# tudoroancea/ihm2

Hardware: AMD Instinct MI355X
Metric: NMPC RTI solves/s (batch), N=40, nx=8 (6-DOF bicycle), fkin6 (higher is better)
Workload: dtype f64

## Files before the change

### ihm2_amd/csrc/kernels_qp.hip

```cpp
#include <cstring>

#include "ihm2mpc_internal.h"
#include "device_steps.hpp"
#include "sqp_body.hpp"
#include "irk_body.hpp"
#include "riccati_mfma.hpp"
#include "sens_body.hpp"
#include "qp_lds.hpp"
#include "qp_mrows.hpp"
#include "qp_reduce.hpp"
#include "qp_catalogue.hpp"
#include "wave_sync.hpp"

using namespace ihm2;

namespace {

#define INF_BOUND 1e20
#ifndef RIC_RING
#define RIC_RING 4
#endif
#ifndef SWEEP_RING
#define SWEEP_RING 4
#endif
#define SWEEP_DL ((SWEEP_RING >= 8) ? 4 : 2)

__device__ __forceinline__ bool fin(double v) { return fabs(v) < INF_BOUND; }
__device__ __forceinline__ int here(int v) { asm volatile("" : "+v"(v)); return v; }

template <typename OP>
__device__ __forceinline__ double wave_reduce(double v, OP op)
{
    v = op(v, dpp_mov<0xB1>(v));
    v = op(v, dpp_mov<0x4E>(v));
    v = op(v, dpp_mov<0x141>(v));
    v = op(v, dpp_mov<0x128>(v));
    int lo = __double2loint(v), hi = __double2hiint(v);
    auto a16 = __builtin_amdgcn_permlane16_swap(lo, lo, false, false);
    auto b16 = __builtin_amdgcn_permlane16_swap(hi, hi, false, false);
    v = op(__hiloint2double(b16[0], a16[0]), __hiloint2double(b16[1], a16[1]));
    lo = __double2loint(v); hi = __double2hiint(v);
    auto a32 = __builtin_amdgcn_permlane32_swap(lo, lo, false, false);
    auto b32 = __builtin_amdgcn_permlane32_swap(hi, hi, false, false);
    return op(__hiloint2double(b32[0], a32[0]), __hiloint2double(b32[1], a32[1]));
}
__device__ __forceinline__ double nanmax(double a, double b) { return (a != a || b != b) ? NAN : fmax(a, b); }
__device__ __forceinline__ double wave_max(double v) { return wave_reduce(v, [](double a, double b) { return fmax(a, b); }); }
__device__ __forceinline__ double wave_min(double v) { return wave_reduce(v, [](double a, double b) { return fmin(a, b); }); }
__device__ __forceinline__ double wave_sum(double v) { return wave_reduce(v, [](double a, double b) { return a + b; }); }
__device__ __forceinline__ double wave_nanmax(double v) { return wave_reduce(v, [](double a, double b) { return nanmax(a, b); }); }
__device__ __forceinline__ void norm_max(double &res, bool &bad, double v) { bad |= v != v; res = fmax(res, v); }

__device__ __forceinline__ double sum8(double v)
{
    v += dpp_mov<0xB1>(v);
    v += dpp_mov<0x4E>(v);
    v += dpp_mov<0x141>(v);
    return v;
}

__device__ __forceinline__ double sum_stride8(double v)
{
    v += dpp_mov<0x128>(v);
// ... 48 lines not shown
                    }
                }
            }
        }
        return;
    }
    double r[2][D], x0[DL], x1[DL];
    const __amdgpu_buffer_rsrc_t rsrc = __builtin_amdgcn_make_buffer_rsrc(const_cast<double *>(rows) - (size_t)QM_PAD * 64, 0, (N + 2 * QM_PAD) * 512, 0x00020000);
    const unsigned ve = (unsigned)e_even * 8u, vo = (unsigned)e_odd * 8u;
    typedef unsigned int u2_t __attribute__((ext_vector_type(2)));
    const double *p_even = rows + (size_t)((DIR < 0) ? N - 1 : 0) * 64 + e_even, *p_odd = rows + (size_t)((DIR < 0) ? N - 1 : 0) * 64 + e_odd;
    auto load_row = [&](const int step, const bool odd) -> double {
        if constexpr (BUF) {
            const int row = (DIR < 0) ? N - 1 - step : step;
            const u2_t v = __builtin_amdgcn_raw_buffer_load_b64(rsrc, odd ? vo : ve, (QM_PAD + row) * 512, 0);
            return __hiloint2double((int)v.y, (int)v.x);
        } else
            return (odd ? p_odd : p_even)[(ptrdiff_t)DIR * step * 64];
    };
#pragma unroll
    for (int d = 0; d < D; d++) {
        r[0][d] = load_row(d, (d & 1) != 0);
        __builtin_amdgcn_sched_barrier(0);
        if (d < DL) pre((DIR < 0) ? N - 1 - d : d, (d & 1) != 0, x0[d], x1[d]);
    }
    for (int s0 = 0; s0 < N; s0 += 2 * D) {
#pragma unroll
        for (int h = 0; h < 2; h++) {
#pragma unroll
            for (int d = 0; d < D; d++) {
                const int s = s0 + h * D + d;
                const int k = (DIR < 0) ? N - 1 - s : s;
                const double v = r[h][d], y0 = x0[d % DL], y1 = x1[d % DL];
                r[h ^ 1][d] = load_row(s + D, (d & 1) != 0);
                pre((DIR < 0) ? k - DL : k + DL, (d & 1) != 0, x0[d % DL], x1[d % DL]);
                if (s < N) body(k, v, (d & 1) != 0, y0, y1);
            }
        }
    }
}
template <int DIR, int D, int DL, typename P, typename F>
__device__ __forceinline__ void stream_rows_v1(const double *rows, int N, int e_even, int e_odd, P &&pre, F &&body)
{
    stream_rows<DIR, D, DL, false>(rows, N, e_even, e_odd, pre, body);
}

template <int NSLOT, int NSOFT, int PATH, int UNI, int NW = 1, int LEAN = 1, int NF = 0, int FULL = 0>
__device__ __forceinline__ void qp_wave_body(const QpArgs &a, const int b, double *sm, const bool want_res = true)
{
    static_assert(NF == 0 || NW == 1, "the straight-line factor sweep parks its idle lanes' stores in the tile the block reductions use");
    static_assert(FULL == 0 || (NSOFT == 0 && PATH == 0 && UNI != 0 && NW == 1 && LEAN != 0 && NF > 0 && NSLOT <= 8),
                  "the full slot form is written for the all-hard table of the batch-shared rows, one wave, the lean phases and the compiled-in horizon");
    constexpr int NT = 64 * NW;
    constexpr bool PAIRM = NF > 0;
    static_assert(!PAIRM || (NF % 4 == 0 && LEAN != 0 && NW == 1 && qm_pair_inside(NF > 0 ? NF : 2, SWEEP_RING, QM_PAD)),
                  "the paired rows: an even horizon in whole factor passes, the lean sweeps, and their unclamped prefetch inside q_M's padding");
    const int tid = threadIdx.x, lane = tid & 63, wv = tid >> 6;
#define BSYNC() do { if (NW == 1) WSYNC(); else __syncthreads(); } while (0)
    const int N = (NF > 0) ? NF : a.N, NS = N + 1;
    constexpr QpLdsClass CLS = qp_lds_class(PATH, UNI != 0);
    constexpr int NCK = CLS.nck;
    const double *Hs0 = a.Hs + (size_t)b * a.hs_bs, *HsT = Hs0 + a.hs_te;
    const double *Gy0 = a.Gy + (size_t)b * a.gy_bs, *GyT = Gy0 + a.gy_te;
    const double *slot_lbb = a.slot_lb + (size_t)b * a.sl_bs, *slot_ubb = a.slot_ub + (size_t)b * a.sl_bs;
    constexpr bool ALAT = PATH == 2;
    constexpr bool HL = CLS.hl, CL = CLS.cl;
    static_assert(qp_factor_inside(qp_lds(40, CLS), 40, NCK) && qp_factor_inside(qp_lds(2, CLS), 2, NCK), "factor stage / block reductions leave their LDS");
    static_assert(qp_sweeps_inside(qp_lds(40, CLS), 40, LEAN != 0, SWEEP_RING, SWEEP_DL) && (LEAN == 0 || qp_sweeps_inside(qp_lds(2, CLS), 2, true, SWEEP_RING, SWEEP_DL)),
                  "the sweeps' unclamped LDS prefetch leaves the block (the earlier form does below N = 4: api.hip refuses those launches)");
    static_assert(NW <= 4, "qp_factor_inside checks the block reductions for four waves");
    static_assert(FULL == 0 || qp_full_zeroes_kept(qp_lds(NF > 0 ? NF : 2, CLS), NF > 0 ? NF : 2), "a store of the factor sweep reaches gam or cf: the full slot form zeroes them once per solve");
#define LEN(id) qp_lds_len(id, N, NS, CLS)
    double *z = sm, *gt = z + LEN(QP_Z), *pi = gt + LEN(QP_GT), *pv = pi + LEN(QP_PI), *rb = pv + LEN(QP_PV), *gam = rb + LEN(QP_RB), *cf = gam + LEN(QP_GAM), *dz = cf + LEN(QP_CF);
    double *kff = dz + LEN(QP_DZ), *Kl = kff + LEN(QP_KFF), *Ginv = Kl + LEN(QP_KL), *Prb = Ginv + LEN(QP_GINV), *tile = Prb + LEN(QP_PRB), *hc = tile + LEN(QP_TILE), *ha = hc + LEN(QP_HC);
    double *Hl = ha + LEN(QP_HA), *CDl = Hl + LEN(QP_HL), *spv = CDl + LEN(QP_CDL);
    int *spc = reinterpret_cast<int *>(spv + 60);
#undef LEN
#define HS(k, i, l) (HL ? Hl[(((k) == N) ? 100 : 0) + (i) * 10 + (l)] : ((k) == N ? HsT : Hs0 + (UNI ? 0 : (k)) * 100)[(i) * 10 + (l)])
#define CDV(k, r, j) (CL ? CDl[(r) * 10 + (j)] : a.CD[((k) * 2 + (r)) * 10 + (j)])

    auto blk_reduce = [&](double v, auto op) -> double {
        v = wave_reduce(v, op);
        if (NW > 1) {
            __syncthreads();
            if (lane == 0) tile[wv] = v;
            __syncthreads();
            v = tile[0];
#pragma unroll
            for (int w = 1; w < NW; w++) v = op(v, tile[w]);
        }
        return v;
    };
    auto blk_max = [&](double v) { return blk_reduce(v, [](double x, double y) { return fmax(x, y); }); };
    auto blk_min = [&](double v) { return blk_reduce(v, [](double x, double y) { return fmin(x, y); }); };
    auto blk_sum = [&](double v) { return blk_reduce(v, [](double x, double y) { return x + y; }); };
    auto blk_nanmax = [&](double v) { return blk_reduce(v, [](double x, double y) { return nanmax(x, y); }); };

    const double *xb = a.x + (size_t)b * NS * 8;
    const double *ub = a.u + (size_t)b * N * 2;
    const double *linb = a.lin + (size_t)b * N * LIN_REC;
    double *gb = a.g + (size_t)b * NS * 10;
    double *rgb = a.rg + (size_t)b * NS * 10;
    double *Pg = a.P + (size_t)b * NS * 64;
    double *Mg = a.M + (size_t)b * N * 64;
    double *pib = a.pi + (size_t)b * NS * 8;
    double *lamb = a.lam + (size_t)b * NS * 28;
// ... 71 lines not shown
            st = fma(-CDV(k, 0, j), lamb[k * 28 + 10] - lamb[k * 28 + 24], st);
            st = fma(-CDV(k, 1, j), lamb[k * 28 + 11] - lamb[k * 28 + 25], st);
        }
        if (PATH && (j == 1 || j == 2)) {
            const double l12 = lamb[k * 28 + 12] - lamb[k * 28 + 26], l13 = lamb[k * 28 + 13] - lamb[k * 28 + 27];
            st -= (j == 1) ? l12 - l13 : hc[k * 2] * l12 + hc[k * 2 + 1] * l13;
        }
        if (ALAT && alat_slot(j) >= 0) st -= ha[k * 4 + alat_slot(j)] * (lamab[k * 2] - lamab[k * 2 + 1]);
        if (counted) r_stat = fmax(r_stat, fabs(st));
    }
    for (int e = tid; e < N * 8; e += NT) {
        const double bl = linb[(size_t)(e / 8) * LIN_REC + 80 + (e % 8)];
        sb = fmax(sb, fabs(bl));
        r_eq = fmax(r_eq, fabs(bl));
    }
    if (tid < 8) {
        const double d = a.x0[(size_t)b * 8 + tid] - xb[tid];
        sb = fmax(sb, fabs(d));
        r_eq = fmax(r_eq, fabs(d));
    }
    if constexpr (FULL != 0) { double sg2 = sg, sb2 = sb; wave_max4(lane, sg, sb, sg2, sb2); }
    else { sg = blk_max(sg); sb = blk_max(sb); }

    int s_kc[NSLOT];
    double s_dl[NSLOT], s_du[NSLOT];
    double lam_l[NSLOT], lam_u[NSLOT], t_l[NSLOT], t_u[NSLOT];
    constexpr int NSO = (NSOFT > 0) ? NSOFT : 1;
    double so_zw[NSO], so_Zw[NSO], so_s[NSO], so_ls[NSO], so_rs[NSO], so_ds[NSO], so_dls[NSO], so_pa[NSO];
#pragma unroll
    for (int r = 0; r < NSO; r++) { so_zw[r] = 0.0; so_Zw[r] = -1.0; so_s[r] = 1.0; so_ls[r] = 0.0; so_rs[r] = 0.0; so_ds[r] = so_dls[r] = so_pa[r] = 0.0; }
#define IS_SOFT(r) ((r) < NSOFT && so_Zw[(r) < NSOFT ? (r) : 0] >= 0.0)
#define ONE_SIDED(r) (NSOFT > 0 && PATH != 2 && (r) < NSOFT)
#define HAS_L(r) (FULL ? true : ONE_SIDED(r) ? true : fin(s_dl[r]))
#define HAS_U(r) (FULL ? true : ONE_SIDED(r) ? false : fin(s_du[r]))
#define ROW_DOT(r, v) (FULL ? row_dot_full((r), (v)) : ONE_SIDED(r) ? s_sg[(r) < NSOFT ? (r) : 0] * row_dot(s_kc[r], (v)) : row_dot(s_kc[r], (v)))
#define NO_SLOT(r) (!FULL && s_kc[r] < 0)
#define SLOT_W(r) (FULL ? (s_kc[r] & 0xffff) >> 3 : s_kc[r])
#define SLOT_AT(arr, r) (*(FULL ? reinterpret_cast<double *>(reinterpret_cast<char *>(arr) + (here(s_kc[r]) & 0xffff)) : &(arr)[s_kc[r]]))
#define ROW_SIGN(r, c) (ONE_SIDED(r) ? s_sg[(r) < NSOFT ? (r) : 0] * (c) : (c))
    double s_sg[NSO];
#pragma unroll
    for (int r = 0; r < NSO; r++) s_sg[r] = 1.0;
#define SLOT_ACC(dst, v) do { if (NSOFT > 0) (dst) += (v); else (dst) = (v); } while (0)
    double r_ineq = 0.0, r_comp = 0.0;
#pragma unroll
    for (int r = 0; r < NSLOT; r++) {
        const int s = tid + NT * r;
        s_kc[r] = FULL ? 0 : -1; s_dl[r] = -INFINITY; s_du[r] = INFINITY;
        lam_l[r] = lam_u[r] = 0.0; t_l[r] = t_u[r] = 1.0;
        const int kc = (s < a.nslots) ? a.slot_kc[s] : -1;
        if (kc >= 0) {
            const int k = kc >> 4, c = kc & 15;
            s_kc[r] = k * NCK + c;
            if (FULL) s_kc[r] = ((k * NCK + c) * 8) | ((k * 10 + ((c < 10) ? c : 0)) << 19) | ((c >= 10) ? (int)(0x80000000u | ((unsigned)(c - 10) << 30)) : 0);
            double cz;
            if (c < 8) cz = xb[k * 8 + c];
            else if (c < 10) cz = ub[k * 2 + c - 8];
            else if (ALAT && c == 14) {
                double g4[4];
                cz = alat_eval(xb[k * 8 + 3], xb[k * 8 + 4], xb[k * 8 + 6], xb[k * 8 + 7], g4);
            } else if (c >= 12) {
                const double n = xb[k * 8 + 1], psi = xb[k * 8 + 2];
                const double foot = -0.5 * a.car_L * sin(fabs(psi)), lat = 0.5 * a.car_W * cos(psi);
                cz = (c == 12) ? n + foot + lat - w_R : -n - foot + lat - w_L;
            } else {
                cz = 0.0;
#pragma unroll
                for (int j = 0; j < 8; j++) cz = fma(CDV(k, c - 10, j), xb[k * 8 + j], cz);
                cz = fma(CDV(k, c - 10, 8), ub[k * 2 + 0], cz);
                cz = fma(CDV(k, c - 10, 9), ub[k * 2 + 1], cz);
            }
            const double lb = slot_lbb[s], ubd = slot_ubb[s];
            bool soft = false;
            if (r < NSOFT) { so_zw[r < NSOFT ? r : 0] = a.slot_zw[s]; so_Zw[r < NSOFT ? r : 0] = a.slot_Zw[s]; soft = a.slot_Zw[s] >= 0.0; }
#define LAM_IN(up) ((ALAT && c == 14) ? lamab[k * 2 + (up)] : lamb[k * 28 + 14 * (up) + c])
            if (fin(lb)) { s_dl[r] = lb - cz; if (want_res && !soft) { r_ineq = fmax(r_ineq, s_dl[r]); r_comp = fmax(r_comp, fabs(LAM_IN(0) * s_dl[r])); } }
            if (fin(ubd)) { s_du[r] = ubd - cz; if (want_res && !soft) { r_ineq = fmax(r_ineq, -s_du[r]); r_comp = fmax(r_comp, fabs(LAM_IN(1) * s_du[r])); } }
#undef LAM_IN
            if (ONE_SIDED(r) && fin(ubd)) { s_sg[r < NSOFT ? r : 0] = -1.0; s_dl[r] = -s_du[r]; }
        }
    }
    if (want_res) {
        if constexpr (FULL != 0) wave_max4(lane, r_stat, r_eq, r_ineq, r_comp);
        else { r_stat = blk_max(r_stat); r_eq = blk_max(r_eq); r_ineq = blk_max(r_ineq); r_comp = blk_max(r_comp); }
    }
    if (want_res && tid == 0) {
        double *rs = a.res + (size_t)b * 4;
        rs[0] = r_stat; rs[1] = r_eq; rs[2] = r_ineq; rs[3] = r_comp;
    }

    const double tol_g = a.tol * sg, tol_b = a.tol * sb, tol_d = a.tol * sb, tol_m = a.tol * sg;
    const double mu_floor = 0.1 * tol_m;
    const double mu0 = a.mu0 * sg;
    const double inv_m = (a.m_act > 0) ? 1.0 / a.m_act : 0.0;

    auto row_dot = [&](int kc, const double *v) -> double {
        const int k = kc / NCK, c = kc % NCK;
        if (c < 10) return v[k * 10 + c];
        if (ALAT && c == 14) return ha[k * 4] * v[k * 10 + 3] + ha[k * 4 + 1] * v[k * 10 + 4] + ha[k * 4 + 2] * v[k * 10 + 6] + ha[k * 4 + 3] * v[k * 10 + 7];
        if (PATH && c >= 12) return (c == 12) ? v[k * 10 + 1] + hc[k * 2] * v[k * 10 + 2] : -v[k * 10 + 1] + hc[k * 2 + 1] * v[k * 10 + 2];
        double acc = 0.0;
#pragma unroll
        for (int j = 0; j < 10; j++) acc = fma(CDV(k, c - 10, j), v[k * 10 + j], acc);
        return acc;
    };
    auto row_dot_full = [&](int r, const double *v) -> double {
        const int pk = here(s_kc[r]);
        const double *vk = reinterpret_cast<const double *>(reinterpret_cast<const char *>(v) + ((pk >> 16) & 0x3fff));
        if (pk >= 0) return vk[0];
        const double *cd = CDl + (((unsigned)pk >> 30) & 1) * 10;
        double acc = 0.0;
#pragma unroll
        for (int j = 0; j < 10; j++) acc = fma(cd[j], vk[j], acc);
        return acc;
    };

    for (int e = tid; e < NS * 10; e += NT) z[e] = (e < 8) ? a.x0[(size_t)b * 8 + e] - xb[e] : 0.0;
    for (int e = tid; e < NS * 8; e += NT) pi[e] = 0.0;
    if (FULL) for (int e = tid; e < NS * NCK; e += NT) { cf[e] = 0.0; gam[e] = 0.0; }
    BSYNC();
#pragma unroll
    for (int r = 0; r < NSLOT; r++) {
        if (NO_SLOT(r)) continue;
        const double rz = ROW_DOT(r, z);
        const bool al = HAS_L(r), au = HAS_U(r);
        double tau_c = a.tau0;
        if (al && au) tau_c = fmin(a.tau0, 0.25 * (s_du[r] - s_dl[r]));
        if (IS_SOFT(r)) {
            const double slack = al ? rz - s_dl[r] : s_du[r] - rz;
            const double s0 = fmax(a.tau0, a.tau0 - slack);
            so_s[r < NSOFT ? r : 0] = s0;
            so_ls[r < NSOFT ? r : 0] = mu0 / s0;
            if (al) { t_l[r] = slack + s0; lam_l[r] = mu0 / t_l[r]; } else { t_u[r] = slack + s0; lam_u[r] = mu0 / t_u[r]; }
            continue;
        }
        if (al) { t_l[r] = fmax(rz - s_dl[r], tau_c); lam_l[r] = mu0 / t_l[r]; }
        if (au) { t_u[r] = fmax(s_du[r] - rz, tau_c); lam_u[r] = mu0 / t_u[r]; }
    }

    int qstatus = 1, it = 0;
    bool exact_mode = false;
    double res_g = 0, res_b = 0, res_d = 0, res_m = 0, mu = 0;
    double fol_g = 0.0, fol_b = 0.0;
    double rd_l[NSLOT], rd_u[NSLOT], dlam_l[NSLOT], dlam_u[NSLOT], dt_l[NSLOT], dt_u[NSLOT];
    double pa_l[NSLOT], pa_u[NSLOT];
    for (it = 0;; it++) {
        bool exact = (it == 0) || exact_mode, finished = false;
        auto multipliers_to_cf = [&]() {
            if (!FULL) {
                for (int e = tid; e < NS * NCK; e += NT) cf[e] = 0.0;
                BSYNC();
            }
#pragma unroll
            for (int r = 0; r < NSLOT; r++) {
                if (NO_SLOT(r)) continue;
                const bool al = HAS_L(r), au = HAS_U(r);
                SLOT_ACC(SLOT_AT(cf, r), ROW_SIGN(r, (al ? lam_l[r] : 0.0) - (au ? lam_u[r] : 0.0)));
            }
            BSYNC();
        };
        if (LEAN != 0) { if (exact) multipliers_to_cf(); }
        else {
            for (int e = tid; e < NS * NCK; e += NT) cf[e] = 0.0;
            BSYNC();
        }
        double mu_acc = 0.0, res_gs = 0.0;
        res_d = 0.0; res_m = 0.0;
        double lane_d = 0.0, lane_m = 0.0;
        bool bad_d = false, bad_m = false, bad_gs = false;
#pragma unroll
        for (int r = 0; r < NSLOT; r++) {
            rd_l[r] = rd_u[r] = 0.0;
            if (NO_SLOT(r)) continue;
            const double rz = ROW_DOT(r, z);
            const bool al = HAS_L(r), au = HAS_U(r);
            const double sv = IS_SOFT(r) ? so_s[r < NSOFT ? r : 0] : 0.0;
            double pl = 0.0, pu = 0.0;
            if constexpr (FULL != 0) {
                rd_l[r] = rz - t_l[r] - s_dl[r] + sv; pl = __dmul_rn(lam_l[r], t_l[r]); norm_max(lane_m, bad_m, fabs(pl));
                rd_u[r] = s_du[r] - rz - t_u[r] + sv; pu = __dmul_rn(lam_u[r], t_u[r]); norm_max(lane_m, bad_m, fabs(pu));
            } else {
            if (al) { rd_l[r] = rz - t_l[r] - s_dl[r] + sv; pl = __dmul_rn(lam_l[r], t_l[r]); res_m = nanmax(res_m, fabs(pl)); }
            if (au) { rd_u[r] = s_du[r] - rz - t_u[r] + sv; pu = __dmul_rn(lam_u[r], t_u[r]); res_m = nanmax(res_m, fabs(pu)); }
            }
            mu_acc = __dadd_rn(mu_acc, __dadd_rn(pl, pu));
            if constexpr (FULL != 0) { bad_d |= __builtin_isunordered(rd_l[r], rd_u[r]); lane_d = fmax(lane_d, fmax(fabs(rd_l[r]), fabs(rd_u[r]))); }
            else
            res_d = nanmax(res_d, nanmax(fabs(rd_l[r]), fabs(rd_u[r])));
            if (IS_SOFT(r)) {
                const int q = r < NSOFT ? r : 0;
                so_rs[q] = so_Zw[q] * so_s[q] + so_zw[q] - (al ? lam_l[r] : lam_u[r]) - so_ls[q];
                if constexpr (FULL != 0) {
                    norm_max(res_gs, bad_gs, fabs(so_rs[q]));
                    mu_acc += so_ls[q] * so_s[q]; norm_max(lane_m, bad_m, fabs(so_ls[q] * so_s[q]));
                } else {
                res_gs = nanmax(res_gs, fabs(so_rs[q]));
                mu_acc += so_ls[q] * so_s[q]; res_m = nanmax(res_m, fabs(so_ls[q] * so_s[q]));
                }
            }
            if (LEAN == 0) SLOT_ACC(SLOT_AT(cf, r), ROW_SIGN(r, (al ? lam_l[r] : 0.0) - (au ? lam_u[r] : 0.0)));
        }
        if constexpr (NW > 1) {
#pragma unroll
            for (int r = 0; r < NSLOT; r++) {
                const int sidx = tid + NT * r;
                if (sidx >= a.nslots_can) continue;
                const bool on = s_kc[r] >= 0;
                gam[sidx] = __dadd_rn((on && fin(s_dl[r])) ? __dmul_rn(lam_l[r], t_l[r]) : 0.0, (on && fin(s_du[r])) ? __dmul_rn(lam_u[r], t_u[r]) : 0.0);
            }
            __syncthreads();
            mu_acc = 0.0;
            for (int sidx = lane; sidx < a.nslots_can; sidx += 64) mu_acc = __dadd_rn(mu_acc, gam[sidx]);
            __syncthreads();
        }
        if (LEAN == 0) BSYNC();
        for (int rpass = 0; rpass < 2; rpass++) {
            if (exact) {
                for (int e = tid; e < NS * 10; e += NT) {
                    const int k = e / 10, j = e % 10;
                    double acc = gb[e];
                    if (HL && h_sparse) {
                        const int row = ((k == N) ? 10 : 0) + j;
// ... 13 lines not shown
                        const double l12 = cf[k * NCK + 12], l13 = cf[k * NCK + 13];
                        acc -= (j == 1) ? l12 - l13 : hc[k * 2] * l12 + hc[k * 2 + 1] * l13;
                    }
                    if (ALAT && alat_slot(j) >= 0) acc -= ha[k * 4 + alat_slot(j)] * cf[k * NCK + 14];
                    gt[e] = acc;
                }
                BSYNC();
                dyn_residual<4, NT>(N, tid, const_cast<double *>(linb), z, pi, gt, rb, LIN_REC);
                BSYNC();
            }
            res_g = 0.0; res_b = 0.0;
            if (exact || LEAN == 0) {
                for (int e = tid; e < NS * 10; e += NT) {
                    const int k = e / 10, j = e % 10;
                    double v = gt[e];
                    if ((k == 0 && j < 8) || (k == N && j >= 8)) { v = 0.0; gt[e] = 0.0; }
                    if (exact) rgb[e] = v;
                    res_g = nanmax(res_g, fabs(v));
                }
                for (int e = tid; e < N * 8; e += NT) res_b = nanmax(res_b, fabs(rb[e]));
            } else { res_g = fol_g; res_b = fol_b; }
            if constexpr (FULL != 0) {
                const bool nan_g = wave_any(res_g != res_g || bad_gs), nan_b = wave_any(res_b != res_b), nan_d = wave_any(bad_d), nan_m = wave_any(bad_m);
                res_g = fmax(res_g, res_gs);
                res_d = lane_d; res_m = lane_m;
                wave_max4(lane, res_g, res_b, res_d, res_m);
                mu = wave_sum(mu_acc) * inv_m;
                res_g = nan_g ? NAN : res_g; res_b = nan_b ? NAN : res_b; res_d = nan_d ? NAN : res_d; res_m = nan_m ? NAN : res_m;
            } else {
            res_g = nanmax(res_g, res_gs);
            res_g = blk_nanmax(res_g); res_b = blk_nanmax(res_b);
            if (rpass == 0) { res_d = blk_nanmax(res_d); res_m = blk_nanmax(res_m); mu = ((NW == 1) ? blk_sum(mu_acc) : wave_sum(mu_acc)) * inv_m; }
            }
            if (!(res_g == res_g) || !(res_b == res_b) || !(res_d == res_d) || !(res_m == res_m)) { qstatus = (it == 0) ? 3 : 4; finished = true; break; }
            const bool conv = res_g <= tol_g && res_b <= tol_b && res_d <= tol_d && res_m <= tol_m;
            if (conv && exact) { qstatus = 0; finished = true; break; }
            if ((conv || it >= a.iter_max) && !exact) {
                exact = true; exact_mode = true;
                if (LEAN != 0) multipliers_to_cf();
                continue;
            }
            break;
        }
        if (finished) break;
        if (it >= a.iter_max) { qstatus = 1; break; }
        BSYNC();
        double alpha = 1.0, alpha_d = 1.0, sigma = 0.0;
        auto slot_coeffs = [&](int pass) {
            if (!FULL) {
                for (int e = tid; e < NS * NCK; e += NT) { cf[e] = 0.0; if (pass == 0) gam[e] = 0.0; }
                BSYNC();
            }
            const double mu_t = fmax(sigma * mu, mu_floor);
#pragma unroll
            for (int r = 0; r < NSLOT; r++) {
                if (NO_SLOT(r)) continue;
                const bool al = HAS_L(r), au = HAS_U(r);
                double c = 0.0;
                if (IS_SOFT(r)) {
                    const int q = r < NSOFT ? r : 0;
                    const double lm = al ? lam_l[r] : lam_u[r], tt = al ? t_l[r] : t_u[r], rdv = al ? rd_l[r] : rd_u[r];
                    const double gm = lm / tt, gs = so_ls[q] / so_s[q], D = so_Zw[q] + gm + gs;
                    double c1, c2, rsv;
                    if (pass == 0) { c1 = (lm * tt + lm * rdv) / tt; c2 = so_ls[q]; rsv = so_rs[q]; SLOT_AT(gam, r) += gm * (so_Zw[q] + gs) / D; }
                    else { c1 = ((al ? pa_l[r] : pa_u[r]) - mu_t) / tt; c2 = (so_pa[q] - mu_t) / so_s[q]; rsv = 0.0; }
                    c = c1 - gm * (rsv + c1 + c2) / D;
                    SLOT_AT(cf, r) += ONE_SIDED(r) ? ROW_SIGN(r, c) : (al ? c : -c);
                    continue;
                }
                if (pass == 0) {
                    const double gl = al ? lam_l[r] / t_l[r] : 0.0, gu = au ? lam_u[r] / t_u[r] : 0.0;
                    if (al) c += fma(gl, rd_l[r], lam_l[r]);
                    if (au) c -= fma(gu, rd_u[r], lam_u[r]);
                    SLOT_ACC(SLOT_AT(gam, r), gl + gu);
                } else {
                    if (al) c += (pa_l[r] - mu_t) / t_l[r];
                    if (au) c -= (pa_u[r] - mu_t) / t_u[r];
                }
                SLOT_ACC(SLOT_AT(cf, r), ROW_SIGN(r, c));
            }
            BSYNC();
        };
        auto add_coeffs = [&]() {
            for (int e = tid; e < NS * 10; e += NT) {
                const int k = e / 10, j = e % 10;
                double acc = gt[e] + cf[k * NCK + j];
                if (k < N) {
                    acc = fma(CDV(k, 0, j), cf[k * NCK + 10], acc);
                    acc = fma(CDV(k, 1, j), cf[k * NCK + 11], acc);
                }
                if (PATH && (j == 1 || j == 2)) {
                    const double c12 = cf[k * NCK + 12], c13 = cf[k * NCK + 13];
                    acc += (j == 1) ? c12 - c13 : hc[k * 2] * c12 + hc[k * 2 + 1] * c13;
                }
                if (ALAT && alat_slot(j) >= 0) acc += ha[k * 4 + alat_slot(j)] * cf[k * NCK + 14];
                gt[e] = acc;
            }
            BSYNC();

        };
        slot_coeffs(0);
        add_coeffs();
        __builtin_amdgcn_s_waitcnt(0x0F70);
        if (wv == 0) {
            RicLds L;
            const QpRic o = qp_lds_ric(N, NS, NCK);
            L.gt = o.gt; L.pv = o.pv; L.gam = o.gam; L.dz = o.dz; L.kff = o.kff; L.Kl = o.Kl;
            L.Ginv = o.Ginv; L.hv = o.Prb; L.tile = o.tile; L.hc = o.hc; L.ha = o.ha;
            if constexpr (NF != 0)
                riccati_sweep_mfma<NCK, PATH != 0, UNI != 0, RIC_RING, ALAT, true, (NF > 0) ? NF : 0>(N, lane, linb, Hs0, HsT, a.CD, L, Pg, Mg, LIN_REC, false, false);
            else
            riccati_sweep_mfma<NCK, PATH != 0, UNI != 0, RIC_RING, ALAT>(N, lane, linb, Hs0, HsT, a.CD, L, Pg, Mg, LIN_REC, a.m_act == 0, a.symmetrize != 0);
            if (lane < 8) dz[lane] = 0.0;
        }
        BSYNC();
        for (int pass = 0; pass < 2; pass++) {
            const double mu_t = fmax(sigma * mu, mu_floor);
            if (pass == 1) slot_coeffs(1);
            if (pass == 1) {
            add_coeffs();
            for (int e = tid; e < NS * 8; e += NT) {
                const int k = e >> 3, j = e & 7;
                double v = gt[k * 10 + j];
                if (k < N) v -= Kl[k * 16 + j] * gt[k * 10 + 8] + Kl[k * 16 + 8 + j] * gt[k * 10 + 9];
                pv[e] = v;
            }
            BSYNC();
            if constexpr (LEAN != 0) {
            if (wv == 0) {
                const int g = lane >> 3, w = lane & 7;
                double pw = pv[N * 8 + w], pg = 0.0;
                const int se2 = (w == 0) ? 16 : 0, so2 = (g == 0) ? 16 : 0;
                const double *be = (w == 0) ? pv + (N - 1) * 8 + g : dz, *bo = (g == 0) ? pv + (N - 2) * 8 + w : dz;
                const double *qe = Prb + (N - 1) * 8 + w, *qo = Prb + (N - 2) * 8 + g;
                double *oe = pv + (N - 1) * 8 + g, *oo = pv + (N - 2) * 8 + w;
                stream_rows<-1, SWEEP_RING, SWEEP_DL, true, PAIRM>(Mg, N, RIC_IDX(w, g), RIC_IDX(g, w),
                    [&](int k, bool odd, double &prb, double &base) {
                        if (odd) { prb = *qo; qo -= 16; base = *bo; bo -= so2; } else { prb = *qe; qe -= 16; base = *be; be -= se2; }
                    },
                    [&](int k, double m, bool odd, double prb, double base) {
                        if (!odd) {
                            pg = sum8(fma(m, pw, fma(m, prb, base)));
                            *oe = pg; oe -= 16;
                        } else {
                            pw = sum_stride8(fma(m, pg, fma(m, prb, base)));
                            *oo = pw; oo -= 16;
                        }
                    });
            }
            } else {
            if (wv == 0) {
                const int g = lane >> 3, w = lane & 7;
                double pw = pv[N * 8 + w], pg = 0.0;
                stream_rows_v1<-1, QP_V1_RING, QP_V1_DL>(Mg, N, RIC_IDX(w, g), RIC_IDX(g, w),
                    [&](int k, bool odd, double &prb, double &base) { prb = Prb[k * 8 + (odd ? g : w)]; base = pv[k * 8 + (odd ? w : g)]; },
                    [&](int k, double m, bool odd, double prb, double base) {
                        if (!odd) {
                            const double off = fma(m, prb, (w == 0) ? base : 0.0);
                            pg = sum8(fma(m, pw, off));
                            if (w == 0) pv[k * 8 + g] = pg;
                        } else {
                            const double off = fma(m, prb, (g == 0) ? base : 0.0);
                            pw = sum_stride8(fma(m, pg, off));
                            if (g == 0) pv[k * 8 + w] = pw;
                        }
                    });
            }
            }
// ... 44 lines not shown
            }
            } else {
            if (wv == 0) {
                const int g = lane >> 3, w = lane & 7;
                double dxw = dz[w], dxg = 0.0;
                stream_rows_v1<+1, QP_V1_RING, QP_V1_DL>(Mg, N, RIC_IDX(g, w), RIC_IDX(w, g),
                    [&](int k, bool odd, double &c, double &unused) { c = dz[(k + 1) * 10 + (odd ? w : g)]; unused = 0.0; },
                    [&](int k, double m, bool odd, double c, double) {
                        if (!odd) {
                            dxg = sum8(fma(m, dxw, (w == 0) ? c : 0.0));
                            if (w == 0) dz[(k + 1) * 10 + g] = dxg;
                        } else {
                            dxw = sum_stride8(fma(m, dxg, (g == 0) ? c : 0.0));
                            if (g == 0) dz[(k + 1) * 10 + w] = dxw;
                        }
                    });
            }
            }
            BSYNC();
            const bool want_dpi = (pass == 1) || (a.m_act == 0);
            for (int e = tid; e < NS * 2; e += NT) {
                const int k = e >> 1, aa = e & 1;
                double acc = 0.0;
                if (k < N) {
                    acc = -kff[k * 4 + aa];
#pragma unroll
                    for (int l = 0; l < 8; l++) acc = fma(-Kl[k * 16 + aa * 8 + l], dz[k * 10 + l], acc);
                }
                dz[k * 10 + 8 + aa] = acc;
            }
            if (want_dpi) {
                const int n = NS * 8;
                for (int base = 0; base < n; base += 3 * NT) {
                    double2 pr[3][4];
#pragma unroll
                    for (int q = 0; q < 3; q++) {
                        const int e = min(base + NT * q + tid, n - 1), k = e >> 3, i = e & 7;
#pragma unroll
                        for (int l = 0; l < 4; l++) pr[q][l] = *reinterpret_cast<const double2 *>(Pg + (size_t)k * 64 + RIC_IDX(l, i));
                    }
#pragma unroll
                    for (int q = 0; q < 3; q++) {
                        const int e = base + NT * q + tid, ec = min(e, n - 1), k = ec >> 3;
                        double acc = pv[ec];
#pragma unroll
                        for (int l = 0; l < 4; l++) { acc = fma(pr[q][l].x, dz[k * 10 + l], acc); acc = fma(pr[q][l].y, dz[k * 10 + l + 4], acc); }
                        if (e < n) pv[e] = acc;
                    }
                }
            }
            BSYNC();

            double amax = 1.0, amax_d = 1.0, mu_aff = 0.0, rmax = 1.0, rmax_d = 1.0;
#pragma unroll
            for (int r = 0; r < NSLOT; r++) {
                dlam_l[r] = dlam_u[r] = dt_l[r] = dt_u[r] = 0.0;
                if (NO_SLOT(r)) continue;
                const double drz = ROW_DOT(r, dz);
                if (IS_SOFT(r)) {
                    const int q = r < NSOFT ? r : 0;
                    const bool al = HAS_L(r);
                    const double lm = al ? lam_l[r] : lam_u[r], tt = al ? t_l[r] : t_u[r], rdv = al ? rd_l[r] : rd_u[r];
                    const double y = al ? drz : -drz;
                    const double gm = lm / tt, gs = so_ls[q] / so_s[q], D = so_Zw[q] + gm + gs;
                    const double rm1 = (pass == 0) ? lm * tt : lm * tt + (al ? pa_l[r] : pa_u[r]) - mu_t;
                    const double rm2 = (pass == 0) ? so_ls[q] * so_s[q] : so_ls[q] * so_s[q] + so_pa[q] - mu_t;
                    const double c1 = (rm1 + lm * rdv) / tt, c2 = rm2 / so_s[q];
                    const double dsv = -(so_rs[q] + c1 + c2) / D - gm / D * y;
                    const double dlsv = -(rm2 + so_ls[q] * dsv) / so_s[q];
                    const double dtv = y + dsv + rdv;
                    const double dlv = -(rm1 + lm * dtv) / tt;
                    so_ds[q] = dsv; so_dls[q] = dlsv;
                    if (al) { dt_l[r] = dtv; dlam_l[r] = dlv; } else { dt_u[r] = dtv; dlam_u[r] = dlv; }
                    if (dsv < 0.0) amax = fmin(amax, -so_s[q] / dsv);
                    if (dlsv < 0.0) amax_d = fmin(amax_d, -so_ls[q] / dlsv);
                    if (dtv < 0.0) amax = fmin(amax, -tt / dtv);
                    if (dlv < 0.0) amax_d = fmin(amax_d, -lm / dlv);
                    continue;
                }
                if (HAS_L(r)) {
                    const double rm = (pass == 0) ? lam_l[r] * t_l[r] : lam_l[r] * t_l[r] + pa_l[r] - mu_t;
                    dt_l[r] = drz + rd_l[r];
                    if (NSOFT == 0) {
                        const double it = 1.0 / t_l[r];
                        dlam_l[r] = -(rm + lam_l[r] * dt_l[r]) * it;
                        rmax = fmax(rmax, -dt_l[r] * it);
                        rmax_d = fmax(rmax_d, -dlam_l[r] / lam_l[r]);
                    } else {
                        dlam_l[r] = -(rm + lam_l[r] * dt_l[r]) / t_l[r];
                        if (dt_l[r] < 0.0) amax = fmin(amax, -t_l[r] / dt_l[r]);
                        if (dlam_l[r] < 0.0) amax_d = fmin(amax_d, -lam_l[r] / dlam_l[r]);
                    }
                }
                if (HAS_U(r)) {
                    const double rm = (pass == 0) ? lam_u[r] * t_u[r] : lam_u[r] * t_u[r] + pa_u[r] - mu_t;
                    dt_u[r] = -drz + rd_u[r];
                    if (NSOFT == 0) {
                        const double it = 1.0 / t_u[r];
                        dlam_u[r] = -(rm + lam_u[r] * dt_u[r]) * it;
                        rmax = fmax(rmax, -dt_u[r] * it);
                        rmax_d = fmax(rmax_d, -dlam_u[r] / lam_u[r]);
                    } else {
                        dlam_u[r] = -(rm + lam_u[r] * dt_u[r]) / t_u[r];
                        if (dt_u[r] < 0.0) amax = fmin(amax, -t_u[r] / dt_u[r]);
                        if (dlam_u[r] < 0.0) amax_d = fmin(amax_d, -lam_u[r] / dlam_u[r]);
                    }
                }
            }
            if (NSOFT == 0) { amax = fmin(amax, 1.0 / rmax); amax_d = fmin(amax_d, 1.0 / rmax_d); }
            if constexpr (FULL != 0) wave_min2(lane, amax, amax_d);
            else { amax = blk_min(amax); amax_d = blk_min(amax_d); }
            if (pass == 0) {
                if (a.m_act == 0) { alpha = alpha_d = 1.0; break; }
#pragma unroll
                for (int r = 0; r < NSLOT; r++) {
                    pa_l[r] = dlam_l[r] * dt_l[r]; pa_u[r] = dlam_u[r] * dt_u[r];
                    if (NO_SLOT(r)) continue;
                    mu_aff = __dadd_rn(mu_aff, __dadd_rn(HAS_L(r) ? __dmul_rn(fma(amax_d, dlam_l[r], lam_l[r]), fma(amax, dt_l[r], t_l[r])) : 0.0,
                                                         HAS_U(r) ? __dmul_rn(fma(amax_d, dlam_u[r], lam_u[r]), fma(amax, dt_u[r], t_u[r])) : 0.0));
                    if (IS_SOFT(r)) {
                        const int q = r < NSOFT ? r : 0;
                        so_pa[q] = so_dls[q] * so_ds[q];
                        mu_aff += (so_ls[q] + amax_d * so_dls[q]) * (so_s[q] + amax * so_ds[q]);
                    }
                }
                if constexpr (NW > 1) {
#pragma unroll
                    for (int r = 0; r < NSLOT; r++) {
                        const int sidx = tid + NT * r;
                        if (sidx >= a.nslots_can) continue;
                        const bool on = s_kc[r] >= 0;
                        gam[sidx] = __dadd_rn((on && fin(s_dl[r])) ? __dmul_rn(fma(amax_d, dlam_l[r], lam_l[r]), fma(amax, dt_l[r], t_l[r])) : 0.0,
                                              (on && fin(s_du[r])) ? __dmul_rn(fma(amax_d, dlam_u[r], lam_u[r]), fma(amax, dt_u[r], t_u[r])) : 0.0);
                    }
                    __syncthreads();
                    mu_aff = 0.0;
                    for (int sidx = lane; sidx < a.nslots_can; sidx += 64) mu_aff = __dadd_rn(mu_aff, gam[sidx]);
                    __syncthreads();
                    mu_aff = wave_sum(mu_aff) * inv_m;
                } else
                mu_aff = blk_sum(mu_aff) * inv_m;
                const double ratio = (mu > 0.0) ? mu_aff / mu : 0.0;
                sigma = ratio * ratio * ratio;
            } else {
                alpha = fmin(1.0, IHM2MPC_IPM_STEP_FRACTION * amax); alpha_d = fmin(1.0, IHM2MPC_IPM_STEP_FRACTION * amax_d);
            }
            BSYNC();
        }
        if (fmin(alpha, alpha_d) < 1e-12) { qstatus = 2; break; }
        if (!exact_mode) {
            const double cd = 1.0 - alpha_d, cp = alpha - alpha_d, cb = 1.0 - alpha;
            const int n10 = NS * 10;
            fol_g = 0.0; fol_b = 0.0;
            for (int base = 0; base < n10; base += 4 * NT) {
                double ro[4];
#pragma unroll
                for (int q = 0; q < 4; q++) ro[q] = rgb[min(base + NT * q + tid, n10 - 1)];
#pragma unroll
                for (int q = 0; q < 4; q++) {
                    const int e = base + NT * q + tid, ec = min(e, n10 - 1), k = ec / 10, j = ec % 10;
                    double hdz = 0.0;
// ... 322 lines not shown
```

### ihm2_amd/csrc/qp_lds.hpp

```cpp
#pragma once

#include <cstddef>

#ifdef __HIPCC__
#define QP_LDS_FN __host__ __device__ constexpr
#else
#define QP_LDS_FN constexpr
#endif

namespace ihm2 {

constexpr int QP_TILE_ROW = 17, QP_TILE_WORDS = 8 * QP_TILE_ROW;
constexpr int QP_V1_RING = 8, QP_V1_DL = 4;
constexpr int QP_DYN_RK4_WORDS = 55;

struct QpLdsClass { int nck; bool hc, ha, hl, cl; };
QP_LDS_FN QpLdsClass qp_lds_class(int path, bool uni) { return {path == 2 ? 15 : path ? 14 : 12, path != 0, path == 2, uni && !path, uni}; }

struct QpArr {
    int off, len;
    QP_LDS_FN operator int() const { return off; }
    QP_LDS_FN int end() const { return off + len; }
};

// ... 58 lines not shown
}

struct QpRic { int gt, pv, gam, dz, kff, Kl, Ginv, Prb, tile, hc, ha; };
QP_LDS_FN QpRic qp_lds_ric(int N, int NS, int nck)
{
    QpRic L = {};
    L.gt = NS * 10; L.pv = NS * 28; L.gam = NS * 36 + N * 8; L.dz = L.gam + 2 * NS * nck; L.kff = L.dz + NS * 10; L.Kl = L.kff + N * 4;
    L.Ginv = L.Kl + N * 16; L.Prb = L.Ginv + N * 8; L.tile = L.Prb + N * 8; L.hc = L.tile + QP_TILE_WORDS; L.ha = L.hc + NS * 2;
    return L;
}
QP_LDS_FN bool qp_lds_ric_agrees(int N, QpLdsClass c)
{
    const QpLds l = qp_lds(N, c);
    const QpRic o = qp_lds_ric(N, N + 1, c.nck);
    return o.gt == l.gt && o.pv == l.pv && o.gam == l.gam && o.dz == l.dz && o.kff == l.kff && o.Kl == l.Kl && o.Ginv == l.Ginv && o.Prb == l.Prb &&
           o.tile == l.tile && o.hc == l.hc && (!c.hc || o.ha == l.ha);
}
QP_LDS_FN bool qp_lds_ric_agrees(int N)
{
    return qp_lds_ric_agrees(N, qp_lds_class(0, false)) && qp_lds_ric_agrees(N, qp_lds_class(0, true)) && qp_lds_ric_agrees(N, qp_lds_class(1, false)) &&
           qp_lds_ric_agrees(N, qp_lds_class(1, true)) && qp_lds_ric_agrees(N, qp_lds_class(2, true));
}
static_assert(qp_lds_ric_agrees(40) && qp_lds_ric_agrees(2), "the factor sweep's offsets are not the layout's");

struct QpReach { int lo, hi; };
QP_LDS_FN bool qp_inside(QpReach r, int lo, int hi) { return lo <= r.lo && r.lo <= r.hi && r.hi <= hi; }

QP_LDS_FN int qp_sweep_fetches(int N, int d, int dl) { return dl + (N + 2 * d - 1) / (2 * d) * 2 * d; }
QP_LDS_FN QpReach qp_reach_lean_vector(const QpLds &l, int N, int d, int dl)
{
    return {l.pv + (N - 2) * 8 - 16 * (qp_sweep_fetches(N, d, dl) / 2 - 1), l.Prb + N * 8};
}
QP_LDS_FN QpReach qp_reach_lean_forward(const QpLds &l, int N, int d, int dl)
{
    return {l.dz, l.dz + 20 + 20 * (qp_sweep_fetches(N, d, dl) / 2 - 1) + 8};
}
QP_LDS_FN QpReach qp_reach_v1_vector(const QpLds &l, int N)
{
    return {l.pv + (N - qp_sweep_fetches(N, QP_V1_RING, QP_V1_DL)) * 8, l.Prb + N * 8};
}
QP_LDS_FN QpReach qp_reach_v1_forward(const QpLds &l, int N)
{
    return {l.dz, l.dz + qp_sweep_fetches(N, QP_V1_RING, QP_V1_DL) * 10 + 8};
}
QP_LDS_FN QpReach qp_reach_plain_parking(const QpLds &l) { return {l.tile, l.tile + 63 + 4 + 1}; }
QP_LDS_FN QpReach qp_reach_plain_operand(const QpLds &l, int N, int nck) { return {l.gt - 10, l.gam + N * nck}; }
QP_LDS_FN QpReach qp_reach_plain_stores(const QpLds &l) { return {l.dz + 10, l.tile.end()}; }
QP_LDS_FN QpReach qp_reach_plain_store_pv(const QpLds &l, int N) { return {l.pv + N * 8, l.pv + N * 8 + 8}; }
QP_LDS_FN bool qp_full_zeroes_kept(const QpLds &l, int N)
{
    const QpReach s = qp_reach_plain_stores(l), p = qp_reach_plain_store_pv(l, N);
    return s.lo >= l.cf.end() && qp_inside(s, l.cf.end(), l.total) && qp_inside(p, 0, l.gam) && l.cf == l.gam.end();
}
QP_LDS_FN QpReach qp_reach_block_reduce(const QpLds &l, int nw) { return {l.tile, l.tile + nw}; }

QP_LDS_FN bool qp_sweeps_inside(const QpLds &l, int N, bool lean, int d, int dl)
{
    return lean ? qp_inside(qp_reach_lean_vector(l, N, d, dl), 0, l.total) && qp_inside(qp_reach_lean_forward(l, N, d, dl), 0, l.total)
                : qp_inside(qp_reach_v1_vector(l, N), 0, l.total) && qp_inside(qp_reach_v1_forward(l, N), 0, l.total);
}
QP_LDS_FN bool qp_factor_inside(const QpLds &l, int N, int nck)
{
    return qp_inside(qp_reach_plain_parking(l), l.tile, l.tile.end()) && qp_inside(qp_reach_block_reduce(l, 4), l.tile, l.tile.end()) &&
           qp_inside(qp_reach_plain_operand(l, N, nck), 0, l.total);
}

constexpr int SENS_ROWS = 15;
QP_LDS_FN size_t sens_factor_lds_doubles(size_t N) { return (N + 1) * (SENS_ROWS + 6) + N * 16 + 64 + 64 + 16 + 100 + 64 + 16 + 84; }
QP_LDS_FN size_t sens_lds_doubles(size_t N) { return sens_factor_lds_doubles(N) + 64 + 16; }
static_assert(sens_lds_doubles(40) == 1989 && sens_lds_doubles(1) == 546, "k_sens: launch LDS at N = 40 and N = 1");

struct StepsLds {
    int qp, sens, dyn_rk4;
    QP_LDS_FN int total() const { return qp > sens ? qp : sens; }
    QP_LDS_FN bool guests_fit() const { return dyn_rk4 <= total(); }
};
QP_LDS_FN StepsLds steps_lds_doubles(int qp_total, int sens_doubles, bool dyn_rk4) { return {qp_total, sens_doubles, dyn_rk4 ? QP_DYN_RK4_WORDS * 64 : 0}; }

}
```

Baseline: 1.315 million.

## Batch slot divisions with AMD div intrinsics and precompute general constraint rows in LDS

For the FULL slot form, the general (polytopic) constraint rows are now evaluated once per phase by all lanes cooperatively into the transpose tile. Each slot's row dot then becomes a single LDS load instead of a per-slot 10-term FMA loop. The per-slot divisions (complementarity coefficients, Newton step dlam, step-length ratios) are also batched through an explicit div_scale/rcp/fma/div_fmas/div_fixup sequence with sched barriers, so independent divisions interleave. The step update is restructured to reuse reciprocals of t. The cost is extra barriers, LDS traffic and register pressure.

```diff
diff --git a/ihm2_amd/csrc/kernels_qp.hip b/ihm2_amd/csrc/kernels_qp.hip
--- a/ihm2_amd/csrc/kernels_qp.hip
+++ b/ihm2_amd/csrc/kernels_qp.hip
@@ -9,6 +9,7 @@
 #include "qp_lds.hpp"
 #include "qp_mrows.hpp"
 #include "qp_reduce.hpp"
+#include "qp_div.hpp"
 #include "qp_catalogue.hpp"
 #include "wave_sync.hpp"
 
@@ -163,6 +164,7 @@
     static_assert(FULL == 0 || (NSOFT == 0 && PATH == 0 && UNI != 0 && NW == 1 && LEAN != 0 && NF > 0 && NSLOT <= 8),
                   "the full slot form is written for the all-hard table of the batch-shared rows, one wave, the lean phases and the compiled-in horizon");
     constexpr int NT = 64 * NW;
+    constexpr int DIVW_RECIP = 5, DIVW_STEP = 5, DIVW_COEFF = 5;
     constexpr bool PAIRM = NF > 0;
     static_assert(!PAIRM || (NF % 4 == 0 && LEAN != 0 && NW == 1 && qm_pair_inside(NF > 0 ? NF : 2, SWEEP_RING, QM_PAD)),
                   "the paired rows: an even horizon in whole factor passes, the lean sweeps, and their unclamped prefetch inside q_M's padding");
@@ -340,7 +342,7 @@
         if (kc >= 0) {
             const int k = kc >> 4, c = kc & 15;
             s_kc[r] = k * NCK + c;
-            if (FULL) s_kc[r] = ((k * NCK + c) * 8) | ((k * 10 + ((c < 10) ? c : 0)) << 19) | ((c >= 10) ? (int)(0x80000000u | ((unsigned)(c - 10) << 30)) : 0);
+            if (FULL) s_kc[r] = qp_full_slot_pack(k, c, NCK);
             double cz;
             if (c < 8) cz = xb[k * 8 + c];
             else if (c < 10) cz = ub[k * 2 + c - 8];
@@ -394,19 +396,30 @@
     };
     auto row_dot_full = [&](int r, const double *v) -> double {
         const int pk = here(s_kc[r]);
-        const double *vk = reinterpret_cast<const double *>(reinterpret_cast<const char *>(v) + ((pk >> 16) & 0x3fff));
-        if (pk >= 0) return vk[0];
-        const double *cd = CDl + (((unsigned)pk >> 30) & 1) * 10;
-        double acc = 0.0;
-#pragma unroll
-        for (int j = 0; j < 10; j++) acc = fma(cd[j], vk[j], acc);
-        return acc;
+        return *reinterpret_cast<const double *>(reinterpret_cast<const char *>(pk < 0 ? tile : v) + ((pk >> 16) & 0x3fff));
+    };
+    static_assert(FULL == 0 || qp_general_rows_inside(qp_lds(NF > 0 ? NF : 2, CLS), NF > 0 ? NF : 2), "the general rows of a phase leave the transpose tile");
+    auto general_rows = [&](const double *v) {
+        for (int e0 = tid; e0 < 2 * N; e0 += 2 * NT) {
+            const bool two = e0 + NT < 2 * N;
+            const double *cd = CDl + (e0 & 1) * 10, *v0 = v + (e0 >> 1) * 10, *v1 = v + ((two ? e0 + NT : e0) >> 1) * 10;
+            double c[10], p[10], q[10];
+#pragma unroll
+            for (int j = 0; j < 10; j++) { c[j] = cd[j]; p[j] = v0[j]; q[j] = v1[j]; }
+            double acc0 = 0.0, acc1 = 0.0;
+#pragma unroll
+            for (int j = 0; j < 10; j++) { acc0 = fma(c[j], p[j], acc0); acc1 = fma(c[j], q[j], acc1); }
+            tile[e0] = acc0;
+            if (two) tile[e0 + NT] = acc1;
+        }
+        BSYNC();
     };
 
     for (int e = tid; e < NS * 10; e += NT) z[e] = (e < 8) ? a.x0[(size_t)b * 8 + e] - xb[e] : 0.0;
     for (int e = tid; e < NS * 8; e += NT) pi[e] = 0.0;
     if (FULL) for (int e = tid; e < NS * NCK; e += NT) { cf[e] = 0.0; gam[e] = 0.0; }
     BSYNC();
+    if constexpr (FULL != 0) general_rows(z);
 #pragma unroll
     for (int r = 0; r < NSLOT; r++) {
         if (NO_SLOT(r)) continue;
@@ -456,6 +469,7 @@
         res_d = 0.0; res_m = 0.0;
         double lane_d = 0.0, lane_m = 0.0;
         bool bad_d = false, bad_m = false, bad_gs = false;
+        if constexpr (FULL != 0) general_rows(z);
 #pragma unroll
         for (int r = 0; r < NSLOT; r++) {
             rd_l[r] = rd_u[r] = 0.0;
@@ -575,6 +589,23 @@
                 BSYNC();
             }
             const double mu_t = fmax(sigma * mu, mu_floor);
+            if constexpr (FULL != 0) {
+                if (pass == 1) {
+                    double cn[2 * NSLOT], cd[2 * NSLOT], cq[2 * NSLOT];
+#pragma unroll
+                    for (int r = 0; r < NSLOT; r++) { cn[2 * r] = pa_l[r] - mu_t; cd[2 * r] = t_l[r]; cn[2 * r + 1] = pa_u[r] - mu_t; cd[2 * r + 1] = t_u[r]; }
+                    div_sets<DIVW_COEFF>(cn, cd, cq);
+#pragma unroll
+                    for (int r = 0; r < NSLOT; r++) {
+                        double c = 0.0;
+                        c += cq[2 * r];
+                        c -= cq[2 * r + 1];
+                        SLOT_AT(cf, r) = c;
+                    }
+                    BSYNC();
+                    return;
+                }
+            }
 #pragma unroll
             for (int r = 0; r < NSLOT; r++) {
                 if (NO_SLOT(r)) continue;
@@ -637,6 +668,15 @@
             if (lane < 8) dz[lane] = 0.0;
         }
         BSYNC();
+        double it_l[NSLOT], it_u[NSLOT];
+        if constexpr (FULL != 0) {
+            double one[2 * NSLOT], tt[2 * NSLOT], rc[2 * NSLOT];
+#pragma unroll
+            for (int r = 0; r < NSLOT; r++) { one[2 * r] = one[2 * r + 1] = 1.0; tt[2 * r] = t_l[r]; tt[2 * r + 1] = t_u[r]; }
+            div_sets<DIVW_RECIP>(one, tt, rc);
+#pragma unroll
+            for (int r = 0; r < NSLOT; r++) { it_l[r] = rc[2 * r]; it_u[r] = rc[2 * r + 1]; }
+        }
         for (int pass = 0; pass < 2; pass++) {
             const double mu_t = fmax(sigma * mu, mu_floor);
             if (pass == 1) slot_coeffs(1);
@@ -787,6 +827,34 @@
             BSYNC();
 
             double amax = 1.0, amax_d = 1.0, mu_aff = 0.0, rmax = 1.0, rmax_d = 1.0;
+            if constexpr (FULL != 0) general_rows(dz);
+            if constexpr (FULL != 0) {
+                double drz[NSLOT], qn[2 * NSLOT], qd[2 * NSLOT], qq[2 * NSLOT];
+#pragma unroll
+                for (int r = 0; r < NSLOT; r++) drz[r] = ROW_DOT(r, dz);
+#pragma unroll
+                for (int r = 0; r < NSLOT; r++) {
+                    {
+                        const double rm = (pass == 0) ? lam_l[r] * t_l[r] : lam_l[r] * t_l[r] + pa_l[r] - mu_t;
+                        dt_l[r] = drz[r] + rd_l[r];
+                        dlam_l[r] = -(rm + lam_l[r] * dt_l[r]) * it_l[r];
+                    }
+                    {
+                        const double rm = (pass == 0) ? lam_u[r] * t_u[r] : lam_u[r] * t_u[r] + pa_u[r] - mu_t;
+                        dt_u[r] = -drz[r] + rd_u[r];
+                        dlam_u[r] = -(rm + lam_u[r] * dt_u[r]) * it_u[r];
+                    }
+                    qn[2 * r] = -dlam_l[r]; qd[2 * r] = lam_l[r]; qn[2 * r + 1] = -dlam_u[r]; qd[2 * r + 1] = lam_u[r];
+                }
+                div_sets<DIVW_STEP>(qn, qd, qq);
+#pragma unroll
+                for (int r = 0; r < NSLOT; r++) {
+                    rmax = fmax(rmax, -dt_l[r] * it_l[r]);
+                    rmax_d = fmax(rmax_d, qq[2 * r]);
+                    rmax = fmax(rmax, -dt_u[r] * it_u[r]);
+                    rmax_d = fmax(rmax_d, qq[2 * r + 1]);
+                }
+            } else
 #pragma unroll
             for (int r = 0; r < NSLOT; r++) {
                 dlam_l[r] = dlam_u[r] = dt_l[r] = dt_u[r] = 0.0;
@@ -842,6 +910,12 @@
                     }
                 }
             }
+            if constexpr (FULL != 0) {
+                const double one[2] = {1.0, 1.0}, rm2[2] = {rmax, rmax_d};
+                double rc[2];
+                div_batch<2>(one, rm2, rc);
+                amax = fmin(amax, rc[0]); amax_d = fmin(amax_d, rc[1]);
+            } else
             if (NSOFT == 0) { amax = fmin(amax, 1.0 / rmax); amax_d = fmin(amax_d, 1.0 / rmax_d); }
             if constexpr (FULL != 0) wave_min2(lane, amax, amax_d);
             else { amax = blk_min(amax); amax_d = blk_min(amax_d); }
diff --git a/ihm2_amd/csrc/qp_div.hpp b/ihm2_amd/csrc/qp_div.hpp
--- /dev/null
+++ b/ihm2_amd/csrc/qp_div.hpp
@@ -0,0 +1,50 @@
+#pragma once
+
+namespace ihm2 {
+
+template <int K, int FENCE = 1>
+__device__ __forceinline__ void div_batch(const double (&num)[K], const double (&den)[K], double (&out)[K])
+{
+#define QP_DIV_STEP(stmt) do { _Pragma("unroll") for (int i = 0; i < K; i++) { stmt; } if (FENCE) __builtin_amdgcn_sched_barrier(0); } while (0)
+    double s0[K], s1[K], r[K], e[K], m[K];
+    bool cc[K];
+    if (FENCE) __builtin_amdgcn_sched_barrier(0);
+    QP_DIV_STEP(bool unused; s0[i] = __builtin_amdgcn_div_scale(num[i], den[i], false, &unused));
+    QP_DIV_STEP(r[i] = __builtin_amdgcn_rcp(s0[i]));
+    QP_DIV_STEP(e[i] = __builtin_fma(-s0[i], r[i], 1.0));
+    QP_DIV_STEP(r[i] = __builtin_fma(r[i], e[i], r[i]));
+    QP_DIV_STEP(e[i] = __builtin_fma(-s0[i], r[i], 1.0));
+    QP_DIV_STEP(s1[i] = __builtin_amdgcn_div_scale(num[i], den[i], true, &cc[i]));
+    QP_DIV_STEP(r[i] = __builtin_fma(r[i], e[i], r[i]));
+    QP_DIV_STEP(m[i] = __dmul_rn(s1[i], r[i]));
+    QP_DIV_STEP(e[i] = __builtin_fma(-s0[i], m[i], s1[i]));
+    QP_DIV_STEP(m[i] = __builtin_amdgcn_div_fmas(e[i], r[i], m[i], cc[i]));
+    QP_DIV_STEP(out[i] = __builtin_amdgcn_div_fixup(m[i], den[i], num[i]));
+#undef QP_DIV_STEP
+}
+
+template <int W, int M, int FENCE = 1>
+__device__ __forceinline__ void div_sets(const double (&num)[M], const double (&den)[M], double (&out)[M])
+{
+    static_assert(W >= 1 && W <= M, "a batch width between 1 and the size of the set");
+#pragma unroll
+    for (int at = 0; at + W <= M; at += W) {
+        double n[W], d[W], q[W];
+#pragma unroll
+        for (int i = 0; i < W; i++) { n[i] = num[at + i]; d[i] = den[at + i]; }
+        div_batch<W, FENCE>(n, d, q);
+#pragma unroll
+        for (int i = 0; i < W; i++) out[at + i] = q[i];
+    }
+    if constexpr (M % W != 0) {
+        constexpr int R = M % W, at = M - R;
+        double n[R], d[R], q[R];
+#pragma unroll
+        for (int i = 0; i < R; i++) { n[i] = num[at + i]; d[i] = den[at + i]; }
+        div_batch<R, FENCE>(n, d, q);
+#pragma unroll
+        for (int i = 0; i < R; i++) out[at + i] = q[i];
+    }
+}
+
+}
diff --git a/ihm2_amd/csrc/qp_lds.hpp b/ihm2_amd/csrc/qp_lds.hpp
--- a/ihm2_amd/csrc/qp_lds.hpp
+++ b/ihm2_amd/csrc/qp_lds.hpp
@@ -134,6 +134,17 @@
     const QpReach s = qp_reach_plain_stores(l), p = qp_reach_plain_store_pv(l, N);
     return s.lo >= l.cf.end() && qp_inside(s, l.cf.end(), l.total) && qp_inside(p, 0, l.gam) && l.cf == l.gam.end();
 }
+QP_LDS_FN QpReach qp_reach_general_rows(const QpLds &l, int N) { return {l.tile, l.tile + 2 * N}; }
+QP_LDS_FN bool qp_general_rows_inside(const QpLds &l, int N) { return qp_inside(qp_reach_general_rows(l, N), l.tile, l.tile.end()); }
+static_assert(qp_general_rows_inside(qp_lds(40, qp_lds_class(0, true)), 40) && qp_general_rows_inside(qp_lds(2, qp_lds_class(0, true)), 2),
+              "the general rows of a phase leave the transpose tile");
+QP_LDS_FN int qp_full_slot_pack(int k, int c, int nck)
+{
+    return ((k * nck + c) * 8) | ((c < 10 ? k * 10 + c : 2 * k + (c - 10)) << 19) | ((c >= 10) ? (int)(0x80000000u | ((unsigned)(c - 10) << 30)) : 0);
+}
+QP_LDS_FN bool qp_full_slot_general(int pk) { return pk < 0; }
+QP_LDS_FN int qp_full_slot_read(int pk) { return (pk >> 16) & 0x3fff; }
+QP_LDS_FN int qp_full_slot_word(int pk) { return pk & 0xffff; }
 QP_LDS_FN QpReach qp_reach_block_reduce(const QpLds &l, int nw) { return {l.tile, l.tile + nw}; }
 
 QP_LDS_FN bool qp_sweeps_inside(const QpLds &l, int N, bool lean, int d, int dl)
```

Measured after the change: 1.377 million (median of 6 runs). 1.05x the previous value.
